# VISION-SJTU/UniDefense

Hardware: AMD Instinct MI355X
Metric: images/sec fwd+bwd (256x256, EffNet-b4) (higher is better)
Workload: dtype f32

## Files before the change

include/unidefense_hip.h:

```cpp
#ifndef UNIDEFENSE_HIP_H
#define UNIDEFENSE_HIP_H
#include <stdint.h>

#ifdef __cplusplus
extern "C" {
#endif

#define UD_EINVAL (-1000)

typedef void* ud_stream_t;

typedef struct {
    int N, Hin, Win, Cin, Hout, Wout, KH, KW, stride, pad_t, pad_l, transposed;
} ud_conv_geom;

typedef struct {
    const float* A; const float* B; float* C;
    int M, N, K;
    long lda, ldb, ldc;
    int a_mode, b_mode, out_mode, split_k;
    int batch; long strideA, strideB, strideC;
    ud_conv_geom g;
    double* stat_sum; double* stat_sumsq;
    int half_mask;
// ... 449 lines not shown
long ud_pj_bwd_fused_grid(int N, int HW, int CE, int CO);
int ud_mb_eval_dw_ok(int Ci, int CE, int K, int stride);
long ud_mb_eval_dw_tiles(int Ho, int Wo, int stride);
int ud_mb_eval_dw(const float* x, const float* we, const ud_bn_ref* bn0, const float* wt, const ud_bn_ref* bn1, float* d, float* part,
                  int N, int H, int W, int Ci, int CE, int Ho, int Wo, int K, int stride, int pad_t, int pad_l, int out_act,
                  ud_stream_t stream);
int ud_mb_eval_dw_h_ok(int Ci, int CE, int K, int stride);
long ud_mb_eval_dw_h_tiles(int Ho, int Wo, int stride);
int ud_mb_eval_dw_h(const void* x, const float* we, const ud_bn_ref* bn0, const float* wt, const ud_bn_ref* bn1, void* d, float* part,
                    int N, int H, int W, int Ci, int CE, int Ho, int Wo, int K, int stride, int pad_t, int pad_l, int out_act,
                    ud_stream_t stream);
int ud_pj_bwd_fused_a(const float* d, const float* dp, const ud_bn_ref* bn, const float* s, const float* w, int N, int HW, int CE,
                      int CO, float* dw, double* dgate, float* part, ud_stream_t stream);
int ud_pj_bwd_fused_b(const float* d, const float* dp, const ud_bn_ref* bn, const float* s, const float* dpool, float inv_hw,
                      const float* w, int N, int HW, int CE, int CO, float* dz, double* s1, double* s2, ud_stream_t stream);
int ud_normbwd_apply_plane_half(const void* x, const void* dy, const float* keep, float inv_keep, const ud_bn_ref* bn,
                                int dy_is_dz, const double* s1, const double* s2, const double* s1_local,
                                const double* s2_local, int G, int R, int C, uint16_t* plane, long panel_stride,
                                float* inv_scale, float* dgamma, float* dbeta, ud_stream_t stream);
int ud_se_bwd_a(const double* dgate, const float* s2, const float* s1, const float* We, double* ds1_acc, float* dWe,
                float* dbe, int N, int C, int Cs, ud_stream_t stream);
int ud_se_bwd_b(const double* ds1_acc, const float* s1, const float* Wr, const double* pool, float pool_scale,
                float* dpool, float* dWr, float* dbr, int N, int C, int Cs, ud_stream_t stream);
int ud_se_scale_bwd_bn(const void* dc, const void* x, const ud_bn_ref* bn, const float* s, const float* dpool,
    float inv_hw, void* dz, double* s1, double* s2, double* ws, int G, int R, int C, int f16, ud_stream_t
    stream);
int ud_coldot_bn_se(const void* dy, const void* x, const ud_bn_ref* bn, int G, int R, int C, double* out, int f16,
                    ud_stream_t stream);
int ud_se_bwd_b_bn(const double* ds1_acc, const float* s1, const float* Wr, const double* pool, float pool_scale,
                   float* dpool, float* dWr, float* dbr, const float* s2, const double* dots, float inv_hw, double* bs1,
// ... 103 lines not shown
```

unidefense_amd/csrc/pjbwd.hip:

```cpp
#include "pw_common.h"

#include <type_traits>

namespace {

using namespace pw;

constexpr int NTH = 256;
constexpr int R = 32;

__device__ __forceinline__ void atomic_add_f64(double* p, double v) { unsafeAtomicAdd(p, v); }

template <int CE, int CO, int CC = CE> struct PjCfg {
    static_assert(CE % CC == 0 && CC % 8 == 0 && (CC % 16 == 0 || CC == CE) && CO % 8 == 0 && CO > 16 && CO <= 64, "thin project convs");
    static constexpr int CCP = (CC + 15) / 16 * 16;
    static constexpr int NCH = CE / CC;
    static constexpr int QT = CE / 4;
    static constexpr int Q = CC / 4;
    static constexpr int NIT = (R * Q + NTH - 1) / NTH;
    static constexpr int RI = (NIT * NTH + Q - 1) / Q;
    static constexpr int NBC = CCP / 16;
    static constexpr int NBW = (NBC + 3) / 4;
    static constexpr int CS = CCP * 2 + 16;
    static constexpr int CP = RI * CS;
    static constexpr int AS = (CCP + 4) * 4;
    static constexpr int AP = RI * AS;
    static constexpr int COP = (CO + 31) / 32 * 32;
    static constexpr int KS2 = COP / 32;
    static constexpr int NB2 = COP / 16;
    static constexpr int DQ = CO / 4;
    static constexpr int NITP = (R * DQ + NTH - 1) / NTH;
    static constexpr int DS = 2 * COP + 16;
    static constexpr int DPL = ((NITP * NTH + DQ - 1) / DQ) * DS;
    static constexpr int COEF = 4 * CC * 4;
    static constexpr int LDS_A = 3 * CP + AP + 3 * DPL + COEF + CC * 4;
    static constexpr int LDS_B = AP + 3 * DPL + COEF + 2 * CC * 4 + 2 * CC * 8;
};

struct PjArgs {
    const float* d;
    const float* dp;
    const float* w;
    const float* s;
    const float* dpool;
    float* dz;
    float* part;
    double* dgate;
    double* s1;
    double* s2;
    const double* bsum;
    const double* bsumsq;
    const float* rmean;
    const float* rvar;
    const float* gamma;
    const float* beta;
    double inv_count;
    float eps;
    float inv_hw;
    int act;
    int HW;
    long M;
    long tiles;
    int gc;
};

__device__ __forceinline__ float act_sel(float z, bool swish) {
    const float sg = ud_sigmoid_fast(z);
    return swish ? z * sg : z;
}
__device__ __forceinline__ float act_grad_sel(float z, bool swish) {
    const float sg = ud_sigmoid_fast(z);
    return swish ? sg * (1.0f + z * (1.0f - sg)) : 1.f;
}

__device__ __forceinline__ void load_coef(const PjArgs& a, float* coef, int c0, int CC, int tid) {
    for (int c = tid; c < CC; c += NTH) {
        double m, v;
        if (a.bsum) {
            m = a.bsum[c0 + c] * a.inv_count;
            v = a.bsumsq[c0 + c] * a.inv_count - m * m;
            if (v < 0.0) v = 0.0;
        } else {
            m = (double)a.rmean[c0 + c];
            v = (double)a.rvar[c0 + c];
        }
        coef[c] = (float)m;
        coef[CC + c] = rsqrtf((float)(v + (double)a.eps));
        coef[2 * CC + c] = a.gamma[c0 + c];
        coef[3 * CC + c] = a.beta[c0 + c];
// ... 7 lines not shown
        const int n = c0 + 16 * min(wave + 4 * j, NBC - 1) + u;
#pragma unroll
        for (int ks = 0; ks < KS2; ++ks) {
            float v[8];
#pragma unroll
            for (int jj = 0; jj < 8; ++jj) {
                const int k = 32 * ks + 8 * g + jj;
                const float wv = w[min(k, CO - 1) * CE + min(n, CE - 1)];
                v[jj] = (k < CO && n < CE) ? wv : 0.f;
            }
            split8(v, wf[j][ks]);
        }
    }
}

template <int CE, int CO, int CC>
__global__ __launch_bounds__(NTH, 2) void pj_bwd_a_kernel(PjArgs a) {
    using CF = PjCfg<CE, CO, CC>;
    extern __shared__ __attribute__((aligned(16))) char L[];
    char* cimg = L;
    char* abuf = L + 3 * CF::CP;
    char* dimg = abuf + CF::AP;
    float* coef = reinterpret_cast<float*>(dimg + 3 * CF::DPL);
    float* gate = coef + 4 * CC;
    const lds_char* Lp = (const lds_char*)L;
    const int tid = threadIdx.x, lane = tid & 63;
    const int wave = __builtin_amdgcn_readfirstlane(tid >> 6);
    const int u = lane & 15, g = lane >> 4, q4 = u >> 2, pp = u & 3;
    const bool swish = a.act == 1;
    const int chunk = blockIdx.x / a.gc, bb = blockIdx.x - chunk * a.gc;
    const int c0 = chunk * CC;

    if constexpr (CF::COP != CO) {
        for (int i = tid; i < 3 * CF::DPL / 16; i += NTH) reinterpret_cast<u32x4*>(dimg)[i] = u32x4{0u, 0u, 0u, 0u};
    }
    if constexpr (CF::CCP != CC) {
        for (int i = tid; i < (3 * CF::CP + CF::AP) / 16; i += NTH) reinterpret_cast<u32x4*>(L)[i] = u32x4{0u, 0u, 0u, 0u};
    }

    f32x4 accw[CF::NBW][CF::NB2];
    double dot[CF::NBW];
#pragma unroll
    for (int j = 0; j < CF::NBW; ++j) {
#pragma unroll
        for (int m = 0; m < CF::NB2; ++m) accw[j][m] = f32x4{0.f, 0.f, 0.f, 0.f};
        dot[j] = 0.0;
    }

    const f32x4* d4 = reinterpret_cast<const f32x4*>(a.d) + chunk * CF::Q;
    const f32x4* dp4 = reinterpret_cast<const f32x4*>(a.dp);
    const long t0 = (long)bb * a.tiles / a.gc, t1 = (long)(bb + 1) * a.tiles / a.gc;
    f32x4 rd[CF::NIT], rp[CF::NITP];
    auto prefetch = [&](long tile_) {
        const long tile = min(tile_, a.tiles - 1);
        const f32x4* db = d4 + tile * (R * CF::QT);
#pragma unroll
        for (int it = 0; it < CF::NIT; ++it) {
            const int idx = tid + it * NTH;
            const int row = idx / CF::Q, q = idx - row * CF::Q;
            rd[it] = db[((it + 1) * NTH <= R * CF::Q || idx < R * CF::Q) ? row * CF::QT + q : 0];
        }
        const f32x4* pb = dp4 + tile * (R * CF::DQ);
#pragma unroll
        for (int it = 0; it < CF::NITP; ++it) {
            const int idx = tid + it * NTH;
            rp[it] = pb[((it + 1) * NTH <= R * CF::DQ || idx < R * CF::DQ) ? idx : 0];
        }
    };
    auto flush = [&](int n) {
        if (g == 0) {
#pragma unroll
            for (int j = 0; j < CF::NBW; ++j)
                if (wave + 4 * j < CF::NBC && 16 * (wave + 4 * j) + u < CC)
                    atomic_add_f64(a.dgate + (long)n * CE + c0 + 16 * (wave + 4 * j) + u, dot[j]);
        }
#pragma unroll
        for (int j = 0; j < CF::NBW; ++j) dot[j] = 0.0;
    };

    prefetch(t0);
    load_coef(a, coef, c0, CC, tid);
    u32x4 wf[CF::NBW][CF::KS2][3];
    load_wfrags<CE, CO, CF::NBC, CF::NBW, CF::KS2>(a.w, c0, wave, u, g, wf);
    int cur_n = -1;
    const f32x4* c4 = reinterpret_cast<const f32x4*>(coef);
    const f32x4* g4 = reinterpret_cast<const f32x4*>(gate);
    __syncthreads();
    for (long tile = t0; tile < t1; ++tile) {
        const int n = (int)(tile * R / a.HW);
        if (n != cur_n) {
            if (cur_n >= 0) flush(cur_n);
            for (int c = tid; c < CC; c += NTH) gate[c] = ud_sigmoid_fast(a.s[(long)n * CE + c0 + c]);
            cur_n = n;
            __syncthreads();
        }
        {
#pragma unroll
            for (int it = 0; it < CF::NIT; ++it) {
                const int idx = tid + it * NTH;
                const int row = idx / CF::Q, q = idx - row * CF::Q;
                const f32x4 mu = c4[q], is = c4[CF::Q + q], ga = c4[2 * CF::Q + q], be = c4[3 * CF::Q + q], gt = g4[q];
                f32x4 av, cv;
#pragma unroll
                for (int k = 0; k < 4; ++k) {
                    const float z = ga[k] * ((rd[it][k] - mu[k]) * is[k]) + be[k];
                    av[k] = act_sel(z, swish);
                    cv[k] = av[k] * gt[k];
                }
                *reinterpret_cast<f32x4*>(abuf + row * CF::AS + q * 16) = av;
                store_split4(cimg + row * CF::CS + q * 8, CF::CP, cv);
            }
#pragma unroll
            for (int it = 0; it < CF::NITP; ++it) {
                const int idx = tid + it * NTH;
                const int row = idx / CF::DQ, q = idx - row * CF::DQ;
                store_split4(dimg + row * CF::DS + q * 8, CF::DPL, rp[it]);
            }
        }
        __syncthreads();
        prefetch(tile + 1);

        {
            const lds_char* drow = Lp + (3 * CF::CP + CF::AP) + u * CF::DS + g * 16;
            Frag3 a0[CF::KS2], a1[CF::KS2];
// ... 1 lines not shown
            for (int ks = 0; ks < CF::KS2; ++ks) {
                a0[ks] = read_rows(drow + ks * 64, CF::DPL);
                a1[ks] = read_rows(drow + 16 * CF::DS + ks * 64, CF::DPL);
            }
            const float* ab = reinterpret_cast<const float*>(abuf) + (4 * g) * (CF::AS / 4) + u;
#pragma unroll
            for (int j = 0; j < CF::NBW; ++j) {
                const int nb = min(wave + 4 * j, CF::NBC - 1);
                f32x4 dc0 = {0.f, 0.f, 0.f, 0.f}, dc1 = {0.f, 0.f, 0.f, 0.f};
#pragma unroll
                for (int ks = 0; ks < CF::KS2; ++ks) {
                    const Frag3 b = frag_of(wf[j][ks]);
                    dc0 = mma6(a0[ks], b, dc0);
                    dc1 = mma6(a1[ks], b, dc1);
                }
                float t = 0.f;
#pragma unroll
                for (int r = 0; r < 4; ++r) {
                    t += dc0[r] * ab[r * (CF::AS / 4) + 16 * nb];
                    t += dc1[r] * ab[(16 + r) * (CF::AS / 4) + 16 * nb];
                }
                t += __shfl_xor(t, 16, 64);
                t += __shfl_xor(t, 32, 64);
                dot[j] += (double)t;
            }
        }
        {
            const lds_char* db = Lp + (3 * CF::CP + CF::AP) + (8 * g + q4) * CF::DS + 4 * pp * 2;
            Frag3 pm[CF::NB2];
#pragma unroll
            for (int m = 0; m < CF::NB2; ++m) pm[m] = read_cols(db + 32 * m, CF::DPL, CF::DS);
            const lds_char* cb = Lp + (8 * g + q4) * CF::CS + 4 * pp * 2;
#pragma unroll
            for (int j = 0; j < CF::NBW; ++j) {
                const int nb = min(wave + 4 * j, CF::NBC - 1);
                const Frag3 b = read_cols(cb + nb * 32, CF::CP, CF::CS);
#pragma unroll
                for (int m = 0; m < CF::NB2; ++m) accw[j][m] = mma6(pm[m], b, accw[j][m]);
            }
// ... 30 lines not shown
        const long st = (long)CO * CC;
        int p = grp;
        for (; p + 16 < gc; p += 32) {
            s0 += src[p * st];
            s1 += src[(p + 16) * st];
        }
        if (p < gc) s0 += src[p * st];
    }
    red[grp][el] = s0 + s1;
    __syncthreads();
    if (grp == 0 && i < numel) {
        float t = red[0][el];
#pragma unroll
        for (int j = 1; j < 16; ++j) t += red[j][el];
        dw[i] = t;
    }
}

template <int CE, int CO, int CC>
__global__ __launch_bounds__(NTH, 2) void pj_bwd_b_kernel(PjArgs a) {
    using CF = PjCfg<CE, CO, CC>;
    extern __shared__ __attribute__((aligned(16))) char L[];
    char* dcbuf = L;
    char* dimg = L + CF::AP;
    float* coef = reinterpret_cast<float*>(dimg + 3 * CF::DPL);
    float* gate = coef + 4 * CC;
    float* dpl = gate + CC;
    double* lacc = reinterpret_cast<double*>(dpl + CC);
    const lds_char* Lp = (const lds_char*)L;
    const int tid = threadIdx.x, lane = tid & 63;
// ... 55 lines not shown
                dpl[c] = a.dpool[(long)n * CE + c0 + c] * a.inv_hw;
            }
            cur_n = n;
        }
#pragma unroll
        for (int it = 0; it < CF::NITP; ++it) {
            const int idx = tid + it * NTH;
            const int row = idx / CF::DQ, q = idx - row * CF::DQ;
            store_split4(dimg + row * CF::DS + q * 8, CF::DPL, rp[it]);
        }
        f32x4 dq[CF::NIT];
#pragma unroll
        for (int it = 0; it < CF::NIT; ++it) dq[it] = rd[it];
        __syncthreads();
        prefetch(tile + 1);
        {
            const lds_char* drow = Lp + CF::AP + u * CF::DS + g * 16;
            Frag3 a0[CF::KS2], a1[CF::KS2];
#pragma unroll
            for (int ks = 0; ks < CF::KS2; ++ks) {
                a0[ks] = read_rows(drow + ks * 64, CF::DPL);
                a1[ks] = read_rows(drow + 16 * CF::DS + ks * 64, CF::DPL);
            }
            float* ob = reinterpret_cast<float*>(dcbuf) + (4 * g) * (CF::AS / 4) + u;
#pragma unroll
            for (int j = 0; j < CF::NBW; ++j) {
                const int nb = min(wave + 4 * j, CF::NBC - 1);
                f32x4 dc0 = {0.f, 0.f, 0.f, 0.f}, dc1 = {0.f, 0.f, 0.f, 0.f};
#pragma unroll
                for (int ks = 0; ks < CF::KS2; ++ks) {
                    const Frag3 b = frag_of(wf[j][ks]);
                    dc0 = mma6(a0[ks], b, dc0);
                    dc1 = mma6(a1[ks], b, dc1);
                }
#pragma unroll
                for (int r = 0; r < 4; ++r) {
                    ob[r * (CF::AS / 4) + 16 * nb] = dc0[r];
                    ob[(16 + r) * (CF::AS / 4) + 16 * nb] = dc1[r];
                }
            }
        }
        __syncthreads();
        {
            f32x4* ob4 = dz4 + tile * (R * CF::QT);
#pragma unroll
            for (int it = 0; it < CF::NIT; ++it) {
                const int idx = tid + it * NTH;
                const int row = idx / CF::Q, q = idx - row * CF::Q;
                const bool ok = (it + 1) * NTH <= R * CF::Q || idx < R * CF::Q;
                const f32x4 mu = c4[q], is = c4[CF::Q + q], ga = c4[2 * CF::Q + q], be = c4[3 * CF::Q + q], gt = g4[q], pl = p4[q];
                const f32x4 dc = *reinterpret_cast<const f32x4*>(dcbuf + row * CF::AS + q * 16);
                f32x4 o;
#pragma unroll
                for (int k = 0; k < 4; ++k) {
                    const float xh = (dq[it][k] - mu[k]) * is[k];
                    float gg = (dc[k] * gt[k] + pl[k]) * act_grad_sel(ga[k] * xh + be[k], swish);
// ... 11 lines not shown
    for (int it = 0; it < CF::NIT; ++it) {
        const int idx = tid + it * NTH;
        if (idx < R * CF::Q) {
            const int q = idx % CF::Q;
#pragma unroll
            for (int k = 0; k < 4; ++k) {
                atomicAdd(&lacc[4 * q + k], (double)sa[it][k]);
                atomicAdd(&lacc[CC + 4 * q + k], (double)sb[it][k]);
            }
        }
    }
    __syncthreads();
    for (int c = tid; c < CC; c += NTH) {
        atomic_add_f64(a.s1 + c0 + c, lacc[c]);
        atomic_add_f64(a.s2 + c0 + c, lacc[CC + c]);
    }
}

template <int CE, int CO> struct PjFwdCfg {
    using B = PjCfg<CE, CO>;
    static constexpr int KD = (CE + 31) / 32 * 32;
    static constexpr int KS = KD / 32;
    static constexpr int CS = KD * 2 + 16;
    static constexpr int CP = B::RI * CS;
    static constexpr int LDS = 3 * CP + B::COEF + CE * 4 + 2 * 4 * 32 * 8;
};

struct PjFwdArgs {
    const float* d;
    const float* w;
// ... 114 lines not shown
            const int nbb = tid >> 4, uu = tid & 15;
            atomic_add_f64(a.sum + tid, wsum[nbb * 16 + uu] + wsum[(2 + nbb) * 16 + uu]);
            atomic_add_f64(a.sumsq + tid, wsum[64 + nbb * 16 + uu] + wsum[64 + (2 + nbb) * 16 + uu]);
        }
    }
}

template <int CE, int CO>
int launch_f(const PjFwdArgs& a, int grid, hipStream_t s) {
    using CF = PjFwdCfg<CE, CO>;
    static_assert(CF::LDS <= 64 * 1024, "dynamic LDS within the default limit");
    hipLaunchKernelGGL((pj_fwd_kernel<CE, CO>), dim3((unsigned)grid), dim3(NTH), CF::LDS, s, a);
    return 0;
}

template <int CE, int CO, int CC>
int launch_a(const PjArgs& a, int grid, hipStream_t s) {
    using CF = PjCfg<CE, CO, CC>;
    static_assert(CF::LDS_A <= 80 * 1024, "two workgroups per CU");
    static bool attr_set = false;
    if (!attr_set) {
        if (hipFuncSetAttribute(reinterpret_cast<const void*>(&pj_bwd_a_kernel<CE, CO, CC>), hipFuncAttributeMaxDynamicSharedMemorySize,
                                CF::LDS_A) != hipSuccess)
            return UD_EINVAL;
        attr_set = true;
    }
    hipLaunchKernelGGL((pj_bwd_a_kernel<CE, CO, CC>), dim3((unsigned)grid), dim3(NTH), CF::LDS_A, s, a);
    return 0;
}
template <int CE, int CO, int CC>
int launch_b(const PjArgs& a, int grid, hipStream_t s) {
    using CF = PjCfg<CE, CO, CC>;
    static_assert(CF::LDS_B <= 64 * 1024, "dynamic LDS within the default limit");
    hipLaunchKernelGGL((pj_bwd_b_kernel<CE, CO, CC>), dim3((unsigned)grid), dim3(NTH), CF::LDS_B, s, a);
    return 0;
}

int chunk_of(int CE, int CO) {
    if (CO == 32 && (CE == 144 || CE == 192)) return CE;
    if (CO == 24 && (CE == 48 || CE == 24)) return CE;
    if (CO == 56 && CE == 336) return 112;
    if (CO == 56 && CE == 192) return 96;
    return 0;
}

bool args_ok(const void* d, const void* dp, const ud_bn_ref* bn, const void* s, const void* w, int N, int HW, int CE, int CO) {
    return d && dp && bn && !ud_bn_eval_form(bn) && s && w && N >= 1 && HW >= R && ud_pj_bwd_fused_ok(CE, CO, HW) && bn->G == 1 && bn->gamma && bn->beta;
}

void fill(PjArgs& a, const float* d, const float* dp, const ud_bn_ref* bn, const float* s, const float* w, int N, int HW, int CE, int CO) {
    a.d = d; a.dp = dp; a.w = w; a.s = s;
    a.bsum = bn->sum; a.bsumsq = bn->sumsq; a.rmean = bn->running_mean; a.rvar = bn->running_var; a.gamma = bn->gamma; a.beta = bn->beta;
    a.inv_count = bn->inv_count; a.eps = bn->eps; a.act = bn->act; a.HW = HW;
    a.M = (long)N * HW; a.tiles = a.M / R;
    a.gc = (int)(ud_pj_bwd_fused_grid(N, HW, CE, CO) / (CE / chunk_of(CE, CO)));
    a.dpool = nullptr; a.dz = nullptr; a.part = nullptr; a.dgate = nullptr; a.s1 = a.s2 = nullptr; a.inv_hw = 0.f;
}

}

extern "C" {

int ud_pj_bwd_fused_ok(int CE, int CO, int HW) { return (chunk_of(CE, CO) && HW >= R && HW % R == 0) ? 1 : 0; }
int ud_pj_fwd_fused_ok(int CE, int CO, int HW) { return (CO <= 32 && chunk_of(CE, CO) == CE && HW >= R && HW % R == 0) ? 1 : 0; }

long ud_pj_bwd_fused_grid(int N, int HW, int CE, int CO) {
    const int cc = chunk_of(CE, CO);
    if (N < 1 || HW < R || HW % R || !cc) return UD_EINVAL;
    const long tiles = (long)N * HW / R, nch = CE / cc, per = 512 / nch;
    return nch * (tiles < per ? tiles : per);
}

int ud_pj_fwd_fused(const float* d, const ud_bn_ref* bn, const float* s, const float* w, int N, int HW, int CE, int CO, float* p,
                     double* sum, double* sumsq, ud_stream_t stream) {
    if (!d || !bn || (!bn->sum && !ud_bn_eval_form(bn)) || !s || !w || !p || N < 1 || !ud_pj_fwd_fused_ok(CE, CO, HW) || bn->G != 1 || !bn->gamma || !bn->beta || (!sum != !sumsq))
        return UD_EINVAL;
    PjFwdArgs a;
    a.d = d; a.w = w; a.s = s; a.p = p; a.sum = sum; a.sumsq = sumsq;
    a.bsum = bn->sum; a.bsumsq = bn->sumsq; a.rmean = bn->running_mean; a.rvar = bn->running_var; a.gamma = bn->gamma; a.beta = bn->beta;
// ... 30 lines not shown
                      const float* w, int N, int HW, int CE, int CO, float* dz, double* s1, double* s2, ud_stream_t stream) {
    if (!args_ok(d, dp, bn, s, w, N, HW, CE, CO) || !dpool || !dz || !s1 || !s2) return UD_EINVAL;
    hipStream_t st = (hipStream_t)stream;
    PjArgs a;
    fill(a, d, dp, bn, s, w, N, HW, CE, CO);
    a.dpool = dpool; a.inv_hw = inv_hw; a.dz = dz; a.s1 = s1; a.s2 = s2;
    const int grid = (int)ud_pj_bwd_fused_grid(N, HW, CE, CO);
    const int rc = CO == 32 ? (CE == 144 ? launch_b<144, 32, 144>(a, grid, st) : launch_b<192, 32, 192>(a, grid, st))
                 : CO == 24 ? (CE == 48 ? launch_b<48, 24, 48>(a, grid, st) : launch_b<24, 24, 24>(a, grid, st))
                            : (CE == 336 ? launch_b<336, 56, 112>(a, grid, st) : launch_b<192, 56, 96>(a, grid, st));
    if (rc) return rc;
    UD_LAUNCH_CHECK();
    return 0;
}

}
```

unidefense_amd/kernels.py:

```python
import ctypes as C
import math
import os

import torch

from . import lib as _lib
from .config import cfg as CFG
from .devmem import Scratch, ZeroPool
from .lib import ConvGeom, GemmDesc, GemmP3Desc

_call = _lib.call
_const, _rows = _lib.const, _lib.const_rows

GEMM_PROFILE = None


def _stream():
    return C.c_void_p(torch.cuda.current_stream().cuda_stream)


def _p(t):
    if t is None:
        return None
    return C.c_void_p(t.data_ptr())
# ... 3059 lines not shown
    grid = _lib.call("ud_pj_bwd_fused_grid", N, HW, Ce, Co)
    part = empty((grid, Co * Ce), d)
    _call("ud_pj_bwd_fused_a", _p(d), _p(dp2), C.byref(bn.ref()), _p(s), _p(w2), N, HW, Ce, Co, _p(dw), _pd(dgate), _p(part), _stream())
    return dw


def project_bwd_fused_b(d, bn, s, dpool, inv_hw, dp2, w2, N, HW, sacc):
    _chk(d, dp2, w2, s, dpool)
    Co, Ce = w2.shape
    dz = torch.empty_like(d)
    _call("ud_pj_bwd_fused_b", _p(d), _p(dp2), C.byref(bn.ref()), _p(s), _p(dpool), float(inv_hw), _p(w2), N, HW, Ce, Co, _p(dz),
          _pd(sacc), _pd(sacc, Ce), _stream())
    return dz


def normbwd_apply_mix(x, dz, bn, G, R, sacc, diff, dalpha_acc, sacc_local=None, energy=None):
    h = _act(x, dz, diff)
    Cc = x.shape[-1]
    loc = sacc if sacc_local is None else sacc_local
    dd = torch.empty_like(x)
    dg = empty((Cc,), x)
    db = empty((Cc,), x)
    _call("ud_normbwd_apply_mix", _p(x), _p(dz), C.byref(bn.ref()), _pd(sacc), _pd(sacc, Cc), _pd(loc), _pd(loc, Cc),
          _p(diff), G, R, Cc, _p(dd), _pd(dalpha_acc), _p(dg), _p(db), _pd(energy) if energy is not None else None, h, _stream())
    return dd, dg, db


def normbwd_apply_se(x, dc, bn, s, dpool, inv_hw, G, R, sacc, sacc_local=None):
    _chk(x, dc, s, dpool)
    assert x.dtype == torch.float32 and dc.dtype == torch.float32
# ... 376 lines not shown
```

unidefense_amd/mbconv.py:

```python
import collections
from types import SimpleNamespace

import torch

from . import kernels as K
from . import tape as T
from .config import cfg


FUSED, HALF, EVAL_NODE, OPERATORS = "fused", "half", "eval_node", "operators"
TrunkMode = collections.namedtuple("TrunkMode", "kind wt dp", defaults=(None,))


_DW_TILED = True


_DW_TILE_OVERRIDE = {}
_DW_BWD_FUSED_OVERRIDE = {}


def _dw_tile_policy(sf, k, stride, H, half):
    ov = _DW_TILE_OVERRIDE.get((bool(sf), k, stride, H, bool(half)))
    if ov is not None and _DW_TILED:
        return ov
# ... 25 lines not shown
    if half:
        return True
    return not (k == 3 and H == 64)


_SE_BN1_FOLD_OVERRIDE = {}


def _se_bn1_fold_policy(sf, stride, Ho, Ce, half):
    if half:
        return False
    ov = _SE_BN1_FOLD_OVERRIDE.get((bool(sf), stride, Ho, Ce))
    if ov is not None:
        return ov
    return True


BlockGeom = collections.namedtuple(
    "BlockGeom", "N H W Cin M k stride pt pl Ho Wo HWo Mo Ce Co Cs We Wsr Wse Wp Wf sf alpha s_f s_i")


def block_geom(blk, x):
    sp = blk.spec
    N, H, W, Cin = x.shape
    Ho, Wo = T.conv_out_hw(H, W, sp.k, sp.stride, sp.pad)
    Ce, Co, Cs = sp.cexp, sp.cout, sp.cse
    sf = sp.sf_norm is not None
    dwm = blk._depthwise_conv
    s_f, s_i = T._fft_scales(H, sp.sf_norm) if sf else (None, None)
    return BlockGeom(N, H, W, Cin, N * H * W, sp.k, sp.stride, sp.pad[2], sp.pad[0], Ho, Wo, Ho * Wo, N * Ho * Wo, Ce, Co, Cs,
# ... 235 lines not shown

def _bwd_project(b, tape, gr):
    g, x, blk, dout = b.geo, b.x, b.blk, gr.dout
    dp_pl = K.normbwd_planes_ok(b.p4, b.pctx)
    sb2 = K.zeros64((3 if dp_pl == 1 else 2) * g.Co, x)
    K.normbwd_sums(b.p4, dout, b.keep, b.inv_keep, b.bn2, False, g.N, g.HWo, sb2)
    loc2 = b.dp.reduce(sb2, keep_local=True)
    gr.dp2, dp_amax, dg2, db2 = _normbwd_to_gemm(b.pctx, dp_pl, b.p4, dout, b.keep, b.inv_keep, b.bn2, False, g.N, g.HWo, sb2, loc2)
    tape.add_param_grad(blk._bn2.weight, dg2)
    tape.add_param_grad(blk._bn2.bias, db2)
    gr.pj_fused = not dp_pl and b.pctx.plans is None and K.project_bwd_fused_ok(b.d, g.Wp, g.HWo)
    assert gr.pj_fused or b.pctx.x is not None, "the fused project forward kept no gated tensor: its backward must be the fused one"
    gr.se_dots = None
    if gr.pj_fused:
        gr.dc = None
        gr.dgate = K.zeros64(g.N * g.Ce, x)
        dWp = K.project_bwd_fused_a(b.d, b.bn1, b.s2, gr.dp2, g.Wp, g.N, g.HWo, gr.dgate)
    else:
        dc, dWp = K.spectral_bwd(b.pctx, gr.dp2, dy_absmax=dp_amax)
        gr.dc = dc.view(g.N, g.Ho, g.Wo, g.Ce)
        if _se_bn1_fold_policy(g.sf, g.stride, g.Ho, g.Ce, b.d.dtype != torch.float32 or dc.dtype != torch.float32):
            gr.se_dots = K.zeros64(5 * g.N * g.Ce, x)
            gr.dgate = gr.se_dots[:g.N * g.Ce]
            K.coldot_bn_se(gr.dc, b.d, b.bn1, g.N, g.HWo, gr.se_dots)
        else:
            gr.dgate = K.zeros64(g.N * g.Ce, x)
            K.coldot_bn(gr.dc, b.d, b.bn1, g.N, g.HWo, gr.dgate)
    tape.add_param_grad(blk._project_conv.weight, dWp)


def _bwd_se(b, tape, gr):
    g, blk = b.geo, b.blk
# ... 4 lines not shown
    tape.add_param_grad(blk._se_expand.bias, dbe2)
    tape.add_param_grad(blk._se_reduce.weight, dWr)
    tape.add_param_grad(blk._se_reduce.bias, dbr)
    gr.dpool = dpool
    if fold is not None:
        gr.dz1 = None
    elif gr.pj_fused:
        gr.dz1 = K.project_bwd_fused_b(b.d, b.bn1, b.s2, dpool, 1.0 / g.HWo, gr.dp2, g.Wp, g.N, g.HWo, gr.sb1)
    else:
        gr.dz1 = K.se_scale_bwd_bn(gr.dc, b.d, b.bn1, b.s2, dpool, 1.0 / g.HWo, g.N, g.HWo, gr.sb1)
    gr.loc1 = b.dp.reduce(gr.sb1, keep_local=True)


def _bn1_apply(b, gr):
    g = b.geo
    if gr.dz1 is None:
        return K.normbwd_apply_se(b.d, gr.dc, b.bn1, b.s2, gr.dpool, 1.0 / g.HWo, g.N, g.HWo, gr.sb1, gr.loc1)
    return K.normbwd_apply(b.d, gr.dz1, None, 1.0, b.bn1, True, g.N, g.HWo, gr.sb1, gr.loc1)


def _bwd_bn1(b, tape, gr):
    g, x, blk, d = b.geo, b.x, b.blk, b.d
    gr.g_alpha, gr.g_mode, gr.da_f, gr.dxf = None, 0, None, None
    if not g.sf:
        gr.g_sp, dg1, db1 = _bn1_apply(b, gr)
    else:
        alpha, sctx = g.alpha, b.sctx
        if g.stride == 1:
            dacc = K.zeros64(64, x)
            dyf_pl = sctx.plans is not None and K.rfft2_planes_ok(d, None)
            en = K.zeros64(g.Ce, x) if dyf_pl else None
            if gr.dz1 is None:
                dd, dg1, db1 = K.normbwd_apply_mix_se(d, gr.dc, b.bn1, b.s2, gr.dpool, 1.0 / g.HWo, g.N, g.HWo, gr.sb1, b.fr, dacc,
                                                      gr.loc1, energy=en)
            else:
                dd, dg1, db1 = K.normbwd_apply_mix(d, gr.dz1, b.bn1, g.N, g.HWo, gr.sb1, b.fr, dacc, gr.loc1, energy=en)
            form = _PLANES if dyf_pl else _PLANE_HALF if (sctx.plans is not None and K.rfft2_plane_half_ok(dd)) else _ROWS
            bound = {"energy": en} if dyf_pl else {}
            dyf, _, dalpha = _rfft2_as(form, dd, g.s_i, 2.0, gate_alpha=alpha, gate_mode=1, gate_acc=dacc, **bound)
            tape.add_param_grad(alpha, dalpha)
            gr.g_sp, gr.g_alpha, gr.g_mode = dd, alpha, 2
        else:
            dd, dg1, db1 = _bn1_apply(b, gr)
            gr.g_sp, dfr, dalpha = K.sfmix_bwd(b.spat, b.fr, alpha, dd, True)
            tape.add_param_grad(alpha, dalpha)
            dyf = K.rfft2(dfr, g.s_i, 2.0, want_absmax=True)
        dyf2, dyf_amax = _gemm_dy(sctx, dyf, dd)
# ... 210 lines not shown
```

Measured before the change: 1473.

## Fold BN1 statistics into fused project backward and add fused BN1 apply kernel

Adds an SE variant of the fused project-conv backward pass A kernel. Besides the gate dot, it accumulates the BN1 backward column statistics (the dz sums and the act-grad/xhat sums), so the separate SE-scale BN backward pass can be skipped. A new pass-C kernel, plus a spectral-mix variant, recomputes dc from dp and the projection weights in registers and applies the BN1 backward directly, without materialising dc or dz. It is enabled only for four listed block geometries and adds recomputation of a small GEMM and more atomics, in exchange for fewer full-tensor reads and writes.

```diff
diff --git a/include/unidefense_hip.h b/include/unidefense_hip.h
--- a/include/unidefense_hip.h
+++ b/include/unidefense_hip.h
@@ -487,6 +487,16 @@
                       int CO, float* dw, double* dgate, float* part, ud_stream_t stream);
 int ud_pj_bwd_fused_b(const float* d, const float* dp, const ud_bn_ref* bn, const float* s, const float* dpool, float inv_hw,
                       const float* w, int N, int HW, int CE, int CO, float* dz, double* s1, double* s2, ud_stream_t stream);
+int ud_pj_bwd_fused_se_ok(int CE, int CO, int HW);
+int ud_pj_bwd_fused_a_se(const float* d, const float* dp, const ud_bn_ref* bn, const float* s, const float* w, int N, int HW, int CE,
+                         int CO, float* dw, double* dots, float* part, ud_stream_t stream);
+int ud_pj_bwd_fused_c(const float* d, const float* dp, const ud_bn_ref* bn, const float* s, const float* dpool, float inv_hw,
+                      const float* w, const double* s1, const double* s2, const double* s1_local, const double* s2_local, int N,
+                      int HW, int CE, int CO, float* dd, float* dgamma, float* dbeta, ud_stream_t stream);
+int ud_pj_bwd_fused_c_mix(const float* d, const float* dp, const ud_bn_ref* bn, const float* s, const float* dpool, float inv_hw,
+                          const float* w, const double* s1, const double* s2, const double* s1_local, const double* s2_local,
+                          const float* diff, int N, int HW, int CE, int CO, float* dd, double* dalpha_acc, float* dgamma,
+                          float* dbeta, double* energy, ud_stream_t stream);
 int ud_normbwd_apply_plane_half(const void* x, const void* dy, const float* keep, float inv_keep, const ud_bn_ref* bn,
                                 int dy_is_dz, const double* s1, const double* s2, const double* s1_local,
                                 const double* s2_local, int G, int R, int C, uint16_t* plane, long panel_stride,
diff --git a/unidefense_amd/csrc/pjbwd.hip b/unidefense_amd/csrc/pjbwd.hip
--- a/unidefense_amd/csrc/pjbwd.hip
+++ b/unidefense_amd/csrc/pjbwd.hip
@@ -35,6 +35,7 @@
     static constexpr int COEF = 4 * CC * 4;
     static constexpr int LDS_A = 3 * CP + AP + 3 * DPL + COEF + CC * 4;
     static constexpr int LDS_B = AP + 3 * DPL + COEF + 2 * CC * 4 + 2 * CC * 8;
+    static constexpr int LDS_C = AP + 3 * DPL + COEF + 4 * CC * 4 + CC * 8 + 4 * 8;
 };
 
 struct PjArgs {
@@ -48,6 +49,17 @@
     double* dgate;
     double* s1;
     double* s2;
+    double* dots;
+    const double* bs1;
+    const double* bs2;
+    const double* bs1l;
+    const double* bs2l;
+    const float* diff;
+    float* dd;
+    float* dgamma;
+    float* dbeta;
+    double* dalpha;
+    double* energy;
     const double* bsum;
     const double* bsumsq;
     const float* rmean;
@@ -73,6 +85,11 @@
     return swish ? sg * (1.0f + z * (1.0f - sg)) : 1.f;
 }
 
+__device__ __forceinline__ float mul_rn(float x, float y) {
+#pragma clang fp contract(off)
+    return x * y;
+}
+
 __device__ __forceinline__ void load_coef(const PjArgs& a, float* coef, int c0, int CC, int tid) {
     for (int c = tid; c < CC; c += NTH) {
         double m, v;
@@ -110,9 +127,11 @@
     }
 }
 
-template <int CE, int CO, int CC>
+template <int CE, int CO, int CC, bool SE = false>
 __global__ __launch_bounds__(NTH, 2) void pj_bwd_a_kernel(PjArgs a) {
     using CF = PjCfg<CE, CO, CC>;
+    static_assert(!SE || CC % 16 == 0, "SE: whole 16-channel blocks (the lane's coefficients are those of a real channel)");
+    constexpr int NS = SE ? 2 : 1;
     extern __shared__ __attribute__((aligned(16))) char L[];
     char* cimg = L;
     char* abuf = L + 3 * CF::CP;
@@ -135,12 +154,13 @@
     }
 
     f32x4 accw[CF::NBW][CF::NB2];
-    double dot[CF::NBW];
+    double dot[CF::NBW][NS];
 #pragma unroll
     for (int j = 0; j < CF::NBW; ++j) {
 #pragma unroll
         for (int m = 0; m < CF::NB2; ++m) accw[j][m] = f32x4{0.f, 0.f, 0.f, 0.f};
-        dot[j] = 0.0;
+#pragma unroll
+        for (int i = 0; i < NS; ++i) dot[j][i] = 0.0;
     }
 
     const f32x4* d4 = reinterpret_cast<const f32x4*>(a.d) + chunk * CF::Q;
@@ -164,14 +184,26 @@
         }
     };
     auto flush = [&](int n) {
-        if (g == 0) {
+        if constexpr (SE) {
+            const long plane = a.M / a.HW * CE;
+#pragma unroll
+            for (int j = 0; j < CF::NBW; ++j) {
+                if (wave + 4 * j < CF::NBC) {
+                    double* o = a.dots + (long)n * CE + c0 + 16 * (wave + 4 * j) + u;
+                    atomic_add_f64(o + g * plane, dot[j][0]);
+                    if (g == 0) atomic_add_f64(o + 4 * plane, dot[j][1]);
+                }
+            }
+        } else if (g == 0) {
 #pragma unroll
             for (int j = 0; j < CF::NBW; ++j)
                 if (wave + 4 * j < CF::NBC && 16 * (wave + 4 * j) + u < CC)
-                    atomic_add_f64(a.dgate + (long)n * CE + c0 + 16 * (wave + 4 * j) + u, dot[j]);
-        }
-#pragma unroll
-        for (int j = 0; j < CF::NBW; ++j) dot[j] = 0.0;
+                    atomic_add_f64(a.dgate + (long)n * CE + c0 + 16 * (wave + 4 * j) + u, dot[j][0]);
+        }
+#pragma unroll
+        for (int j = 0; j < CF::NBW; ++j)
+#pragma unroll
+            for (int i = 0; i < NS; ++i) dot[j][i] = 0.0;
     };
 
     prefetch(t0);
@@ -182,6 +214,14 @@
     const f32x4* c4 = reinterpret_cast<const f32x4*>(coef);
     const f32x4* g4 = reinterpret_cast<const f32x4*>(gate);
     __syncthreads();
+    float lmu[CF::NBW], lis[CF::NBW], lga[CF::NBW], lbe[CF::NBW];
+    if constexpr (SE) {
+#pragma unroll
+        for (int j = 0; j < CF::NBW; ++j) {
+            const int c = 16 * min(wave + 4 * j, CF::NBC - 1) + u;
+            lmu[j] = coef[c]; lis[j] = coef[CC + c]; lga[j] = coef[2 * CC + c]; lbe[j] = coef[3 * CC + c];
+        }
+    }
     for (long tile = t0; tile < t1; ++tile) {
         const int n = (int)(tile * R / a.HW);
         if (n != cur_n) {
@@ -203,7 +243,7 @@
                     av[k] = act_sel(z, swish);
                     cv[k] = av[k] * gt[k];
                 }
-                *reinterpret_cast<f32x4*>(abuf + row * CF::AS + q * 16) = av;
+                *reinterpret_cast<f32x4*>(abuf + row * CF::AS + q * 16) = SE ? rd[it] : av;
                 store_split4(cimg + row * CF::CS + q * 8, CF::CP, cv);
             }
 #pragma unroll
@@ -235,15 +275,42 @@
                     dc0 = mma6(a0[ks], b, dc0);
                     dc1 = mma6(a1[ks], b, dc1);
                 }
-                float t = 0.f;
+                float t = 0.f, ta1 = 0.f, ta2 = 0.f, tb1 = 0.f, tb2 = 0.f;
 #pragma unroll
                 for (int r = 0; r < 4; ++r) {
-                    t += dc0[r] * ab[r * (CF::AS / 4) + 16 * nb];
-                    t += dc1[r] * ab[(16 + r) * (CF::AS / 4) + 16 * nb];
+#pragma unroll
+                    for (int h = 0; h < 2; ++h) {
+                        const float dcv = h ? dc1[r] : dc0[r];
+                        const float tv = ab[(16 * h + r) * (CF::AS / 4) + 16 * nb];
+                        if constexpr (SE) {
+                            const float xh = (tv - lmu[j]) * lis[j];
+                            const float z = lga[j] * xh + lbe[j];
+                            const float ap = act_grad_sel(z, swish);
+                            const float uu = mul_rn(dcv, ap);
+                            t += mul_rn(dcv, act_sel(z, swish));
+                            ta1 += uu;
+                            ta2 += uu * xh;
+                            tb1 += ap;
+                            tb2 += ap * xh;
+                        } else {
+                            t += mul_rn(dcv, tv);
+                        }
+                    }
                 }
-                t += __shfl_xor(t, 16, 64);
-                t += __shfl_xor(t, 32, 64);
-                dot[j] += (double)t;
+                if constexpr (SE) {
+                    t += __shfl_xor(t, 16, 64);     t += __shfl_xor(t, 32, 64);
+                    ta1 += __shfl_xor(ta1, 16, 64); ta1 += __shfl_xor(ta1, 32, 64);
+                    ta2 += __shfl_xor(ta2, 16, 64); ta2 += __shfl_xor(ta2, 32, 64);
+                    tb1 += __shfl_xor(tb1, 16, 64); tb1 += __shfl_xor(tb1, 32, 64);
+                    tb2 += __shfl_xor(tb2, 16, 64); tb2 += __shfl_xor(tb2, 32, 64);
+                    const float lo = (g & 1) ? ta1 : t, hi = (g & 1) ? tb1 : ta2;
+                    dot[j][0] += (double)((g & 2) ? hi : lo);
+                    dot[j][1] += (double)tb2;
+                } else {
+                    t += __shfl_xor(t, 16, 64);
+                    t += __shfl_xor(t, 32, 64);
+                    dot[j][0] += (double)t;
+                }
             }
         }
         {
@@ -304,6 +371,35 @@
 #pragma unroll
         for (int j = 1; j < 16; ++j) t += red[j][el];
         dw[i] = t;
+    }
+}
+
+template <typename CF>
+__device__ __forceinline__ void dc_tile_to_lds(const lds_char* dimg, char* dcbuf, const u32x4 (&wf)[CF::NBW][CF::KS2][3], int wave,
+                                               int u, int g) {
+    const lds_char* drow = dimg + u * CF::DS + g * 16;
+    Frag3 a0[CF::KS2], a1[CF::KS2];
+#pragma unroll
+    for (int ks = 0; ks < CF::KS2; ++ks) {
+        a0[ks] = read_rows(drow + ks * 64, CF::DPL);
+        a1[ks] = read_rows(drow + 16 * CF::DS + ks * 64, CF::DPL);
+    }
+    float* ob = reinterpret_cast<float*>(dcbuf) + (4 * g) * (CF::AS / 4) + u;
+#pragma unroll
+    for (int j = 0; j < CF::NBW; ++j) {
+        const int nb = min(wave + 4 * j, CF::NBC - 1);
+        f32x4 dc0 = {0.f, 0.f, 0.f, 0.f}, dc1 = {0.f, 0.f, 0.f, 0.f};
+#pragma unroll
+        for (int ks = 0; ks < CF::KS2; ++ks) {
+            const Frag3 b = frag_of(wf[j][ks]);
+            dc0 = mma6(a0[ks], b, dc0);
+            dc1 = mma6(a1[ks], b, dc1);
+        }
+#pragma unroll
+        for (int r = 0; r < 4; ++r) {
+            ob[r * (CF::AS / 4) + 16 * nb] = dc0[r];
+            ob[(16 + r) * (CF::AS / 4) + 16 * nb] = dc1[r];
+        }
     }
 }
 
@@ -389,32 +485,7 @@
         for (int it = 0; it < CF::NIT; ++it) dq[it] = rd[it];
         __syncthreads();
         prefetch(tile + 1);
-        {
-            const lds_char* drow = Lp + CF::AP + u * CF::DS + g * 16;
-            Frag3 a0[CF::KS2], a1[CF::KS2];
-#pragma unroll
-            for (int ks = 0; ks < CF::KS2; ++ks) {
-                a0[ks] = read_rows(drow + ks * 64, CF::DPL);
-                a1[ks] = read_rows(drow + 16 * CF::DS + ks * 64, CF::DPL);
-            }
-            float* ob = reinterpret_cast<float*>(dcbuf) + (4 * g) * (CF::AS / 4) + u;
-#pragma unroll
-            for (int j = 0; j < CF::NBW; ++j) {
-                const int nb = min(wave + 4 * j, CF::NBC - 1);
-                f32x4 dc0 = {0.f, 0.f, 0.f, 0.f}, dc1 = {0.f, 0.f, 0.f, 0.f};
-#pragma unroll
-                for (int ks = 0; ks < CF::KS2; ++ks) {
-                    const Frag3 b = frag_of(wf[j][ks]);
-                    dc0 = mma6(a0[ks], b, dc0);
-                    dc1 = mma6(a1[ks], b, dc1);
-                }
-#pragma unroll
-                for (int r = 0; r < 4; ++r) {
-                    ob[r * (CF::AS / 4) + 16 * nb] = dc0[r];
-                    ob[(16 + r) * (CF::AS / 4) + 16 * nb] = dc1[r];
-                }
-            }
-        }
+        dc_tile_to_lds<CF>(Lp + CF::AP, dcbuf, wf, wave, u, g);
         __syncthreads();
         {
             f32x4* ob4 = dz4 + tile * (R * CF::QT);
@@ -456,6 +527,164 @@
     for (int c = tid; c < CC; c += NTH) {
         atomic_add_f64(a.s1 + c0 + c, lacc[c]);
         atomic_add_f64(a.s2 + c0 + c, lacc[CC + c]);
+    }
+}
+
+template <int CE, int CO, int CC, bool MIX>
+__global__ __launch_bounds__(NTH, 2) void pj_bwd_c_kernel(PjArgs a) {
+    using CF = PjCfg<CE, CO, CC>;
+    extern __shared__ __attribute__((aligned(16))) char L[];
+    char* dcbuf = L;
+    char* dimg = L + CF::AP;
+    float* coef = reinterpret_cast<float*>(dimg + 3 * CF::DPL);
+    float* gate = coef + 4 * CC;
+    float* dpl = gate + CC;
+    float* tt = dpl + CC;
+    double* eacc = reinterpret_cast<double*>(tt + 2 * CC);
+    double* wsum = eacc + CC;
+    const lds_char* Lp = (const lds_char*)L;
+    const int tid = threadIdx.x, lane = tid & 63;
+    const int wave = __builtin_amdgcn_readfirstlane(tid >> 6);
+    const int u = lane & 15, g = lane >> 4;
+    const bool swish = a.act == 1;
+    const int chunk = blockIdx.x / a.gc, bb = blockIdx.x - chunk * a.gc;
+    const int c0 = chunk * CC;
+
+    if constexpr (CF::COP != CO) {
+        for (int i = tid; i < 3 * CF::DPL / 16; i += NTH) reinterpret_cast<u32x4*>(dimg)[i] = u32x4{0u, 0u, 0u, 0u};
+    }
+    for (int c = tid; c < CC; c += NTH) {
+        tt[c] = (float)a.bs1[c0 + c] * (float)a.inv_count;
+        tt[CC + c] = (float)a.bs2[c0 + c] * (float)a.inv_count;
+        if constexpr (MIX) eacc[c] = 0.0;
+    }
+
+    const f32x4* d4 = reinterpret_cast<const f32x4*>(a.d) + chunk * CF::Q;
+    const f32x4* f4 = MIX ? reinterpret_cast<const f32x4*>(a.diff) + chunk * CF::Q : nullptr;
+    const f32x4* dp4 = reinterpret_cast<const f32x4*>(a.dp);
+    f32x4* dd4 = reinterpret_cast<f32x4*>(a.dd) + chunk * CF::Q;
+    const long t0 = (long)bb * a.tiles / a.gc, t1 = (long)(bb + 1) * a.tiles / a.gc;
+    f32x4 rd[CF::NIT], rp[CF::NITP], rf[MIX ? CF::NIT : 1];
+    auto prefetch = [&](long tile_) {
+        const long tile = min(tile_, a.tiles - 1);
+        const f32x4* db = d4 + tile * (R * CF::QT);
+        const f32x4* fb = MIX ? f4 + tile * (R * CF::QT) : nullptr;
+#pragma unroll
+        for (int it = 0; it < CF::NIT; ++it) {
+            const int idx = tid + it * NTH;
+            const int row = idx / CF::Q, q = idx - row * CF::Q;
+            const int o = ((it + 1) * NTH <= R * CF::Q || idx < R * CF::Q) ? row * CF::QT + q : 0;
+            rd[it] = db[o];
+            if constexpr (MIX) rf[it] = fb[o];
+        }
+        const f32x4* pb = dp4 + tile * (R * CF::DQ);
+#pragma unroll
+        for (int it = 0; it < CF::NITP; ++it) {
+            const int idx = tid + it * NTH;
+            rp[it] = pb[((it + 1) * NTH <= R * CF::DQ || idx < R * CF::DQ) ? idx : 0];
+        }
+    };
+
+    prefetch(t0);
+    load_coef(a, coef, c0, CC, tid);
+    u32x4 wf[CF::NBW][CF::KS2][3];
+    load_wfrags<CE, CO, CF::NBC, CF::NBW, CF::KS2>(a.w, c0, wave, u, g, wf);
+    double acc = 0.0;
+    float en[MIX ? CF::NIT : 1][4];
+#pragma unroll
+    for (int it = 0; it < (MIX ? CF::NIT : 1); ++it)
+#pragma unroll
+        for (int k = 0; k < 4; ++k) en[it][k] = 0.f;
+    auto en_flush = [&]() {
+#pragma unroll
+        for (int it = 0; it < (MIX ? CF::NIT : 1); ++it) {
+            const int idx = tid + it * NTH;
+            if (idx < R * CF::Q) {
+                const int q = idx % CF::Q;
+#pragma unroll
+                for (int k = 0; k < 4; ++k) atomicAdd(&eacc[4 * q + k], (double)en[it][k] * 1.0001);
+            }
+#pragma unroll
+            for (int k = 0; k < 4; ++k) en[it][k] = 0.f;
+        }
+    };
+    int cur_n = -1;
+    const f32x4* c4 = reinterpret_cast<const f32x4*>(coef);
+    const f32x4* g4 = reinterpret_cast<const f32x4*>(gate);
+    const f32x4* p4 = reinterpret_cast<const f32x4*>(dpl);
+    const f32x4* t4 = reinterpret_cast<const f32x4*>(tt);
+    __syncthreads();
+    for (long tile = t0; tile < t1; ++tile) {
+        const int n = (int)(tile * R / a.HW);
+        if (n != cur_n) {
+            __syncthreads();
+            for (int c = tid; c < CC; c += NTH) {
+                gate[c] = ud_sigmoid_fast(a.s[(long)n * CE + c0 + c]);
+                dpl[c] = a.dpool[(long)n * CE + c0 + c] * a.inv_hw;
+            }
+            cur_n = n;
+        }
+#pragma unroll
+        for (int it = 0; it < CF::NITP; ++it) {
+            const int idx = tid + it * NTH;
+            const int row = idx / CF::DQ, q = idx - row * CF::DQ;
+            store_split4(dimg + row * CF::DS + q * 8, CF::DPL, rp[it]);
+        }
+        f32x4 dq[CF::NIT], fq[MIX ? CF::NIT : 1];
+#pragma unroll
+        for (int it = 0; it < CF::NIT; ++it) {
+            dq[it] = rd[it];
+            if constexpr (MIX) fq[it] = rf[it];
+        }
+        __syncthreads();
+        prefetch(tile + 1);
+        dc_tile_to_lds<CF>(Lp + CF::AP, dcbuf, wf, wave, u, g);
+        __syncthreads();
+        {
+            f32x4* ob4 = dd4 + tile * (R * CF::QT);
+#pragma unroll
+            for (int it = 0; it < CF::NIT; ++it) {
+                const int idx = tid + it * NTH;
+                const int row = idx / CF::Q, q = idx - row * CF::Q;
+                const bool ok = (it + 1) * NTH <= R * CF::Q || idx < R * CF::Q;
+                const f32x4 mu = c4[q], is = c4[CF::Q + q], ga = c4[2 * CF::Q + q], be = c4[3 * CF::Q + q], gt = g4[q], pl = p4[q];
+                const f32x4 ta = t4[q], tb = t4[CF::Q + q];
+                const f32x4 dc = *reinterpret_cast<const f32x4*>(dcbuf + row * CF::AS + q * 16);
+                f32x4 o;
+#pragma unroll
+                for (int k = 0; k < 4; ++k) {
+                    const float xh = (dq[it][k] - mu[k]) * is[k];
+                    const float dz = mul_rn(dc[k] * gt[k] + pl[k], act_grad_sel(ga[k] * xh + be[k], swish));
+                    const float ov = mul_rn(ga[k], is[k]) * __builtin_fmaf(-xh, tb[k], dz - ta[k]);
+                    o[k] = ok ? ov : 0.f;
+                    if constexpr (MIX) {
+                        acc += (double)o[k] * (double)fq[it][k];
+                        en[it][k] += o[k] * o[k];
+                    }
+                }
+                if (ok) ob4[row * CF::QT + q] = o;
+            }
+        }
+        if constexpr (MIX) {
+            if (a.energy && ((tile - t0) & 63) == 63) en_flush();
+        }
+    }
+    if (bb == 0) {
+        for (int c = tid; c < CC; c += NTH) {
+            if (a.dbeta) a.dbeta[c0 + c] = (float)a.bs1l[c0 + c];
+            if (a.dgamma) a.dgamma[c0 + c] = (float)a.bs2l[c0 + c];
+        }
+    }
+    if constexpr (MIX) {
+        if (a.energy) {
+            en_flush();
+            __syncthreads();
+            for (int c = tid; c < CC; c += NTH) atomic_add_f64(a.energy + c0 + c, eacc[c]);
+        }
+        acc = ud_wave_sum_d(acc);
+        if (lane == 0) wsum[wave] = acc;
+        __syncthreads();
+        if (tid == 0) atomic_add_f64(a.dalpha + (blockIdx.x & 63), (wsum[0] + wsum[1]) + (wsum[2] + wsum[3]));
     }
 }
 
@@ -600,18 +829,18 @@
     return 0;
 }
 
-template <int CE, int CO, int CC>
+template <int CE, int CO, int CC, bool SE = false>
 int launch_a(const PjArgs& a, int grid, hipStream_t s) {
     using CF = PjCfg<CE, CO, CC>;
     static_assert(CF::LDS_A <= 80 * 1024, "two workgroups per CU");
     static bool attr_set = false;
     if (!attr_set) {
-        if (hipFuncSetAttribute(reinterpret_cast<const void*>(&pj_bwd_a_kernel<CE, CO, CC>), hipFuncAttributeMaxDynamicSharedMemorySize,
+        if (hipFuncSetAttribute(reinterpret_cast<const void*>(&pj_bwd_a_kernel<CE, CO, CC, SE>), hipFuncAttributeMaxDynamicSharedMemorySize,
                                 CF::LDS_A) != hipSuccess)
             return UD_EINVAL;
         attr_set = true;
     }
-    hipLaunchKernelGGL((pj_bwd_a_kernel<CE, CO, CC>), dim3((unsigned)grid), dim3(NTH), CF::LDS_A, s, a);
+    hipLaunchKernelGGL((pj_bwd_a_kernel<CE, CO, CC, SE>), dim3((unsigned)grid), dim3(NTH), CF::LDS_A, s, a);
     return 0;
 }
 template <int CE, int CO, int CC>
@@ -620,6 +849,18 @@
     static_assert(CF::LDS_B <= 64 * 1024, "dynamic LDS within the default limit");
     hipLaunchKernelGGL((pj_bwd_b_kernel<CE, CO, CC>), dim3((unsigned)grid), dim3(NTH), CF::LDS_B, s, a);
     return 0;
+}
+template <int CE, int CO, int CC, bool MIX>
+int launch_c(const PjArgs& a, int grid, hipStream_t s) {
+    using CF = PjCfg<CE, CO, CC>;
+    static_assert(CF::LDS_C <= 64 * 1024, "dynamic LDS within the default limit");
+    hipLaunchKernelGGL((pj_bwd_c_kernel<CE, CO, CC, MIX>), dim3((unsigned)grid), dim3(NTH), CF::LDS_C, s, a);
+    return 0;
+}
+template <bool MIX>
+int launch_c_of(const PjArgs& a, int CE, int CO, int grid, hipStream_t st) {
+    return CO == 32 ? (CE == 144 ? launch_c<144, 32, 144, MIX>(a, grid, st) : launch_c<192, 32, 192, MIX>(a, grid, st))
+                    : (CE == 336 ? launch_c<336, 56, 112, MIX>(a, grid, st) : launch_c<192, 56, 96, MIX>(a, grid, st));
 }
 
 int chunk_of(int CE, int CO) {
@@ -641,6 +882,20 @@
     a.M = (long)N * HW; a.tiles = a.M / R;
     a.gc = (int)(ud_pj_bwd_fused_grid(N, HW, CE, CO) / (CE / chunk_of(CE, CO)));
     a.dpool = nullptr; a.dz = nullptr; a.part = nullptr; a.dgate = nullptr; a.s1 = a.s2 = nullptr; a.inv_hw = 0.f;
+    a.dots = nullptr; a.bs1 = a.bs2 = a.bs1l = a.bs2l = nullptr; a.diff = nullptr; a.dd = nullptr; a.dgamma = a.dbeta = nullptr;
+    a.dalpha = a.energy = nullptr;
+}
+
+bool c_args_ok(const void* d, const void* dp, const ud_bn_ref* bn, const void* s, const void* dpool, const void* w, const double* s1,
+               const double* s2, const double* s1_local, const double* s2_local, int N, int HW, int CE, int CO, const void* dd,
+               const float* dgamma, const float* dbeta) {
+    return args_ok(d, dp, bn, s, w, N, HW, CE, CO) && ud_pj_bwd_fused_se_ok(CE, CO, HW) && dpool && s1 && s2 && dd &&
+           !((dgamma || dbeta) && (!s1_local || !s2_local));
+}
+void fill_c(PjArgs& a, const float* dpool, float inv_hw, const double* s1, const double* s2, const double* s1_local,
+            const double* s2_local, float* dd, float* dgamma, float* dbeta) {
+    a.dpool = dpool; a.inv_hw = inv_hw; a.bs1 = s1; a.bs2 = s2; a.bs1l = s1_local; a.bs2l = s2_local; a.dd = dd; a.dgamma = dgamma;
+    a.dbeta = dbeta;
 }
 
 }
@@ -649,6 +904,8 @@
 
 int ud_pj_bwd_fused_ok(int CE, int CO, int HW) { return (chunk_of(CE, CO) && HW >= R && HW % R == 0) ? 1 : 0; }
 int ud_pj_fwd_fused_ok(int CE, int CO, int HW) { return (CO <= 32 && chunk_of(CE, CO) == CE && HW >= R && HW % R == 0) ? 1 : 0; }
+
+int ud_pj_bwd_fused_se_ok(int CE, int CO, int HW) { return (ud_pj_bwd_fused_ok(CE, CO, HW) && CO != 24) ? 1 : 0; }
 
 long ud_pj_bwd_fused_grid(int N, int HW, int CE, int CO) {
     const int cc = chunk_of(CE, CO);
@@ -709,4 +966,50 @@
     return 0;
 }
 
-}
+int ud_pj_bwd_fused_a_se(const float* d, const float* dp, const ud_bn_ref* bn, const float* s, const float* w, int N, int HW, int CE,
+                         int CO, float* dw, double* dots, float* part, ud_stream_t stream) {
+    if (!args_ok(d, dp, bn, s, w, N, HW, CE, CO) || !ud_pj_bwd_fused_se_ok(CE, CO, HW) || !dw || !dots || !part) return UD_EINVAL;
+    hipStream_t st = (hipStream_t)stream;
+    PjArgs a;
+    fill(a, d, dp, bn, s, w, N, HW, CE, CO);
+    a.part = part; a.dots = dots;
+    const int grid = (int)ud_pj_bwd_fused_grid(N, HW, CE, CO);
+    const int rc = CO == 32 ? (CE == 144 ? launch_a<144, 32, 144, true>(a, grid, st) : launch_a<192, 32, 192, true>(a, grid, st))
+                            : (CE == 336 ? launch_a<336, 56, 112, true>(a, grid, st) : launch_a<192, 56, 96, true>(a, grid, st));
+    if (rc) return rc;
+    UD_LAUNCH_CHECK();
+    hipLaunchKernelGGL(pj_fold_kernel, dim3((unsigned)ud_cdiv((long)CO * CE, 16)), dim3(256), 0, st, part, a.gc, CO, CE, chunk_of(CE, CO), dw);
+    UD_LAUNCH_CHECK();
+    return 0;
+}
+
+int ud_pj_bwd_fused_c(const float* d, const float* dp, const ud_bn_ref* bn, const float* s, const float* dpool, float inv_hw,
+                      const float* w, const double* s1, const double* s2, const double* s1_local, const double* s2_local, int N,
+                      int HW, int CE, int CO, float* dd, float* dgamma, float* dbeta, ud_stream_t stream) {
+    if (!c_args_ok(d, dp, bn, s, dpool, w, s1, s2, s1_local, s2_local, N, HW, CE, CO, dd, dgamma, dbeta)) return UD_EINVAL;
+    PjArgs a;
+    fill(a, d, dp, bn, s, w, N, HW, CE, CO);
+    fill_c(a, dpool, inv_hw, s1, s2, s1_local, s2_local, dd, dgamma, dbeta);
+    const int rc = launch_c_of<false>(a, CE, CO, (int)ud_pj_bwd_fused_grid(N, HW, CE, CO), (hipStream_t)stream);
+    if (rc) return rc;
+    UD_LAUNCH_CHECK();
+    return 0;
+}
+
+int ud_pj_bwd_fused_c_mix(const float* d, const float* dp, const ud_bn_ref* bn, const float* s, const float* dpool, float inv_hw,
+                          const float* w, const double* s1, const double* s2, const double* s1_local, const double* s2_local,
+                          const float* diff, int N, int HW, int CE, int CO, float* dd, double* dalpha_acc, float* dgamma,
+                          float* dbeta, double* energy, ud_stream_t stream) {
+    if (!c_args_ok(d, dp, bn, s, dpool, w, s1, s2, s1_local, s2_local, N, HW, CE, CO, dd, dgamma, dbeta) || !diff || !dalpha_acc)
+        return UD_EINVAL;
+    PjArgs a;
+    fill(a, d, dp, bn, s, w, N, HW, CE, CO);
+    fill_c(a, dpool, inv_hw, s1, s2, s1_local, s2_local, dd, dgamma, dbeta);
+    a.diff = diff; a.dalpha = dalpha_acc; a.energy = energy;
+    const int rc = launch_c_of<true>(a, CE, CO, (int)ud_pj_bwd_fused_grid(N, HW, CE, CO), (hipStream_t)stream);
+    if (rc) return rc;
+    UD_LAUNCH_CHECK();
+    return 0;
+}
+
+}
diff --git a/unidefense_amd/kernels.py b/unidefense_amd/kernels.py
--- a/unidefense_amd/kernels.py
+++ b/unidefense_amd/kernels.py
@@ -3097,6 +3097,50 @@
     return dz
 
 
+def project_bwd_fold_ok(w2, HW):
+    return _lib.call("ud_pj_bwd_fused_se_ok", int(w2.shape[1]), int(w2.shape[0]), int(HW)) == 1
+
+
+def project_bwd_fused_a_se(d, bn, s, dp2, w2, N, HW, dots):
+    _chk(d, dp2, w2, s)
+    Co, Ce = w2.shape
+    assert d.numel() == N * HW * Ce and dp2.numel() == N * HW * Co and s.numel() == N * Ce and dp2.is_contiguous()
+    assert dots.numel() >= 5 * N * Ce
+    dw = empty((Co, Ce), d)
+    grid = _lib.call("ud_pj_bwd_fused_grid", N, HW, Ce, Co)
+    part = empty((grid, Co * Ce), d)
+    _call("ud_pj_bwd_fused_a_se", _p(d), _p(dp2), C.byref(bn.ref()), _p(s), _p(w2), N, HW, Ce, Co, _p(dw), _pd(dots), _p(part),
+          _stream())
+    return dw
+
+
+def project_bwd_fused_c(d, bn, s, dpool, inv_hw, dp2, w2, N, HW, sacc, sacc_local=None):
+    _chk(d, dp2, w2, s, dpool)
+    Co, Ce = w2.shape
+    loc = sacc if sacc_local is None else sacc_local
+    dd = torch.empty_like(d)
+    dg = empty((Ce,), d)
+    db = empty((Ce,), d)
+    _call("ud_pj_bwd_fused_c", _p(d), _p(dp2), C.byref(bn.ref()), _p(s), _p(dpool), float(inv_hw), _p(w2), _pd(sacc), _pd(sacc, Ce),
+          _pd(loc), _pd(loc, Ce), N, HW, Ce, Co, _p(dd), _p(dg), _p(db), _stream())
+    dd._ud_absmax = None
+    return dd, dg, db
+
+
+def project_bwd_fused_c_mix(d, bn, s, dpool, inv_hw, dp2, w2, N, HW, sacc, diff, dalpha_acc, sacc_local=None, energy=None):
+    _chk(d, dp2, w2, s, dpool, diff)
+    assert diff.dtype == torch.float32 and diff.numel() == d.numel()
+    Co, Ce = w2.shape
+    loc = sacc if sacc_local is None else sacc_local
+    dd = torch.empty_like(d)
+    dg = empty((Ce,), d)
+    db = empty((Ce,), d)
+    _call("ud_pj_bwd_fused_c_mix", _p(d), _p(dp2), C.byref(bn.ref()), _p(s), _p(dpool), float(inv_hw), _p(w2), _pd(sacc),
+          _pd(sacc, Ce), _pd(loc), _pd(loc, Ce), _p(diff), N, HW, Ce, Co, _p(dd), _pd(dalpha_acc), _p(dg), _p(db),
+          _pd(energy) if energy is not None else None, _stream())
+    return dd, dg, db
+
+
 def normbwd_apply_mix(x, dz, bn, G, R, sacc, diff, dalpha_acc, sacc_local=None, energy=None):
     h = _act(x, dz, diff)
     Cc = x.shape[-1]
diff --git a/unidefense_amd/mbconv.py b/unidefense_amd/mbconv.py
--- a/unidefense_amd/mbconv.py
+++ b/unidefense_amd/mbconv.py
@@ -63,6 +63,18 @@
     if ov is not None:
         return ov
     return True
+
+
+_PJ_BN1_FOLD_OVERRIDE = {}
+_PJ_BN1_FOLD_RULE = {(False, 2, 64, 144): True, (False, 1, 64, 192): True, (True, 2, 32, 192): True, (True, 1, 32, 336): True}
+
+
+def _pj_bn1_fold_policy(sf, stride, Ho, Ce):
+    key = (bool(sf), stride, Ho, Ce)
+    ov = _PJ_BN1_FOLD_OVERRIDE.get(key)
+    if ov is not None:
+        return ov
+    return _PJ_BN1_FOLD_RULE.get(key, False)
 
 
 BlockGeom = collections.namedtuple(
@@ -328,8 +340,13 @@
     gr.se_dots = None
     if gr.pj_fused:
         gr.dc = None
-        gr.dgate = K.zeros64(g.N * g.Ce, x)
-        dWp = K.project_bwd_fused_a(b.d, b.bn1, b.s2, gr.dp2, g.Wp, g.N, g.HWo, gr.dgate)
+        if K.project_bwd_fold_ok(g.Wp, g.HWo) and _pj_bn1_fold_policy(g.sf, g.stride, g.Ho, g.Ce):
+            gr.se_dots = K.zeros64(5 * g.N * g.Ce, x)
+            gr.dgate = gr.se_dots[:g.N * g.Ce]
+            dWp = K.project_bwd_fused_a_se(b.d, b.bn1, b.s2, gr.dp2, g.Wp, g.N, g.HWo, gr.se_dots)
+        else:
+            gr.dgate = K.zeros64(g.N * g.Ce, x)
+            dWp = K.project_bwd_fused_a(b.d, b.bn1, b.s2, gr.dp2, g.Wp, g.N, g.HWo, gr.dgate)
     else:
         dc, dWp = K.spectral_bwd(b.pctx, gr.dp2, dy_absmax=dp_amax)
         gr.dc = dc.view(g.N, g.Ho, g.Wo, g.Ce)
@@ -364,6 +381,8 @@
 
 def _bn1_apply(b, gr):
     g = b.geo
+    if gr.dz1 is None and gr.dc is None:
+        return K.project_bwd_fused_c(b.d, b.bn1, b.s2, gr.dpool, 1.0 / g.HWo, gr.dp2, g.Wp, g.N, g.HWo, gr.sb1, gr.loc1)
     if gr.dz1 is None:
         return K.normbwd_apply_se(b.d, gr.dc, b.bn1, b.s2, gr.dpool, 1.0 / g.HWo, g.N, g.HWo, gr.sb1, gr.loc1)
     return K.normbwd_apply(b.d, gr.dz1, None, 1.0, b.bn1, True, g.N, g.HWo, gr.sb1, gr.loc1)
@@ -380,7 +399,10 @@
             dacc = K.zeros64(64, x)
             dyf_pl = sctx.plans is not None and K.rfft2_planes_ok(d, None)
             en = K.zeros64(g.Ce, x) if dyf_pl else None
-            if gr.dz1 is None:
+            if gr.dz1 is None and gr.dc is None:
+                dd, dg1, db1 = K.project_bwd_fused_c_mix(d, b.bn1, b.s2, gr.dpool, 1.0 / g.HWo, gr.dp2, g.Wp, g.N, g.HWo, gr.sb1,
+                                                         b.fr, dacc, gr.loc1, energy=en)
+            elif gr.dz1 is None:
                 dd, dg1, db1 = K.normbwd_apply_mix_se(d, gr.dc, b.bn1, b.s2, gr.dpool, 1.0 / g.HWo, g.N, g.HWo, gr.sb1, b.fr, dacc,
                                                       gr.loc1, energy=en)
             else:
```

Result: faster. 1489 (median of 6 runs) (+1.1%).
